# pyranha-labs/hypergrep

Hardware: NVIDIA B200
Metric: scanned GB/s (higher is better)
Workload: dtype u8

## Files before the change

### hypergrep_b200/csrc/capi.cpp

```cpp
#include <cuda_runtime.h>
#include <sys/stat.h>

#include <algorithm>
#include <atomic>
#include <chrono>
#include <cstdio>
#include <cstdlib>
#include <cstring>
#include <condition_variable>
#include <functional>
#include <list>
#include <mutex>
#include <thread>
#include <utility>
#include <string>
#include <vector>

#include "../../include/gpugrep.h"
#include "database.hpp"
#include "engine.hpp"
#include "ingest.hpp"

namespace gpugrep {
void set_last_error(const std::string& e);
// ... 240 lines not shown
    std::vector<uint32_t> report_end_flat;

    bool limit_reached() const { return max_match > 0 && out->count() >= max_match; }

    int deliver(const SegmentResult& r, const uint8_t* host, ScanSlot* slot) {
        stats.lines += r.num_lines;
        stats.gpu_ms += r.stats.gpu_ms;
        stats.stream_kernel_ms += r.stats.stream_ms;
        stats.launches += r.stats.launches;
        stats.stream_launches += r.stats.stream_launches;
        stats.candidates += r.stats.candidates;
        stats.h2d_bytes += r.stats.h2d_bytes;
        stats.d2h_bytes += r.stats.d2h_bytes;
        stats.path |= r.stats.path;
        stats.segments++;
        if (stop) return 0;
        int rc = db->simple ? deliver_simple(r, host, slot) : deliver_events(r, host, slot);
        line_base += r.num_lines;
        return rc;
    }

    int deliver_simple(const SegmentResult& r, const uint8_t* host, ScanSlot* slot) {
        const LineRec* recs = r.lines;
        size_t count = r.num_line_recs;
        const bool fast_rec = (r.stats.path & 1) != 0;
        if (fast_rec) {
            if (!out->wants_lines() && max_match == 0) { out->emit_count_only(r.num_valid_recs); return 0; }
            if (r.num_valid_recs != count) {
                unique_.clear();
                unique_.reserve(r.num_valid_recs);
// ... 578 lines not shown
            spec.count_only = count_only;
            std::memset(&stats[g], 0, sizeof(gpugrep_stats));
            rcs[g] = spec.end > spec.begin ? run(g, spec, &stats[g]) : 0;
            if (rcs[g]) errors[g] = gpugrep_last_error();
        });
    }
    for (auto& w : workers) w.join();
    gpugrep_stats total;
    std::memset(&total, 0, sizeof(total));
    for (size_t g = 0; g < G; g++) {
        if (rcs[g]) { set_last_error(errors[g]); return rcs[g]; }
        total.bytes_scanned += stats[g].bytes_scanned; total.lines += stats[g].lines; total.candidates += stats[g].candidates;
        total.h2d_bytes += stats[g].h2d_bytes; total.d2h_bytes += stats[g].d2h_bytes; total.gpu_ms += stats[g].gpu_ms;
        total.stream_kernel_ms += stats[g].stream_kernel_ms; total.launches += stats[g].launches;
        total.stream_launches += stats[g].stream_launches; total.segments += stats[g].segments; total.path |= stats[g].path;
    }
    Deliverer out(pr.cb, effective_batch(pr));
    unsigned long long line_base = 0;
    bool stop = false;
    for (size_t g = 0; g < G && !stop; g++) {
        if (count_only) {
            out.emit_count_only(stats[g].matches);
        } else {
            const auto& recs = results[g].records;
            for (size_t i = 0; i < recs.size() && !stop;) {
                size_t j = i;
                for (; j < recs.size() && recs[j].line == recs[i].line; j++) {
                    if (pr.cb) out.emit_text(recs[j].id, line_base + recs[j].line, results[g].text.data() + recs[j].offset);
                    else out.emit_count_only(1);
                }
// ... 169 lines not shown
```

### hypergrep_b200/csrc/device_types.cuh

```cuda
#pragma once

namespace gpugrep {

struct GroupDev {
    const uint16_t* trans;
    const uint8_t* cls;
    const uint32_t* accept_of;
    const uint16_t* flat;
    const uint16_t* eod_next;
    const uint16_t* ctab;
    const uint8_t* cmap;
    uint32_t crow, cstates;
    const uint8_t* depth;
    uint32_t cdepth_off;
    uint32_t stride, eod, first_accept, dead, accept_base, idle_end, mid_other, mid_word;
};

struct DbView {
    const GroupDev* groups;
    int ngroups;
    const NfaView* nfas;
    int nnfa;
};

constexpr uint32_t kInvalidLen = 0xffffffffu;
constexpr uint32_t kHasNulBit = 0x80000000u;

struct Totals {
    unsigned long long meta_total;
    unsigned long long rec_total;
    unsigned long long aux_total;
    unsigned int flags;
    unsigned int last_byte;
    unsigned int max_line;
    unsigned int survivors;
};

#define CUDA_TRY(expr)                                                                      \
    do {                                                                                    \
        cudaError_t e_ = (expr);                                                            \
        if (e_ != cudaSuccess) {                                                            \
// ... 7 lines not shown
```

### hypergrep_b200/csrc/engine.cu

```cuda
#include <cuda_runtime.h>

#include <algorithm>
#include <cstdio>
#include <cstdlib>
#include <cstring>
#include <mutex>
#include <unordered_map>
#include <vector>

#include "engine.hpp"
#include "nfa_sim.hpp"

#include "device_types.cuh"
#include "swar.cuh"
#include "confirm.cuh"
#include "k_stream.cuh"
#include "scan.cuh"
#include "dfa_walk.cuh"
#include "k_fast.cuh"
#include "k_general.cuh"
#include "k_invert.cuh"

namespace gpugrep {

// ... 399 lines not shown
}

template <class Load>
static void launch_scan(cudaStream_t st, Load load, size_t n, unsigned long long* out, unsigned long long* sums, unsigned long long* total,
                        SegmentStats& stats, const unsigned long long* limit = nullptr, int limit_shift = 32) {
    size_t nb = (n + kScanTile - 1) / kScanTile;
    if (nb == 0) nb = 1;
    static const unsigned per_sm = blocks_per_sm(k_scan_sums<Load>, kScanThreads);
    unsigned grid = (unsigned)std::min<size_t>(nb, (size_t)per_sm * device_sms());
    k_scan_sums<Load><<<grid, kScanThreads, 0, st>>>(load, n, sums, nb, limit, limit_shift);
    k_scan_top<<<1, 1024, 0, st>>>(sums, nb, total);
    k_scan_write<Load><<<grid, kScanThreads, 0, st>>>(load, n, sums, out, nb, limit, limit_shift);
    stats.launches += 3;
}

template <int STRIDE, bool FOLD, int MODE, int NODD = 0>
static cudaError_t launch_stream_t(cudaStream_t st, int grid, int block, size_t smem, const uint8_t* data, size_t n, unsigned long long* meta,
                                   uint32_t* nlmask, unsigned long long* gsum, const DevicePrefilter* pf) {
    if (smem > 48 * 1024) {
        cudaError_t e = cudaFuncSetAttribute(k_stream<STRIDE, FOLD, MODE, NODD>, cudaFuncAttributeMaxDynamicSharedMemorySize, (int)smem);
        if (e != cudaSuccess) return e;
    }
    k_stream<STRIDE, FOLD, MODE, NODD><<<grid, block, smem, st>>>(data, n, meta, nlmask, gsum, pf ? pf->d_table : nullptr, pf ? pf->table_words : 0,
                                                            pf ? pf->pp : ProbeParams{});
    return cudaGetLastError();
}

template <int MODE>
static cudaError_t launch_stream_m(cudaStream_t st, int grid, int block, size_t smem, const uint8_t* data, size_t n, unsigned long long* meta,
                                   uint32_t* nlmask, unsigned long long* gsum, const DevicePrefilter* pf) {
    int key = pf->stride * 2 + (pf->fold ? 1 : 0);
    if (MODE == 2 && pf->stride == 4 && pf->nodd > 0)
        return pf->fold ? launch_stream_t<4, true, MODE, 2>(st, grid, block, smem, data, n, meta, nlmask, gsum, pf)
                        : launch_stream_t<4, false, MODE, 2>(st, grid, block, smem, data, n, meta, nlmask, gsum, pf);
    switch (key) {
        case 8: return launch_stream_t<4, false, MODE>(st, grid, block, smem, data, n, meta, nlmask, gsum, pf);
        case 9: return launch_stream_t<4, true, MODE>(st, grid, block, smem, data, n, meta, nlmask, gsum, pf);
        case 4: return launch_stream_t<2, false, MODE>(st, grid, block, smem, data, n, meta, nlmask, gsum, pf);
        case 5: return launch_stream_t<2, true, MODE>(st, grid, block, smem, data, n, meta, nlmask, gsum, pf);
        case 2: return launch_stream_t<1, false, MODE>(st, grid, block, smem, data, n, meta, nlmask, gsum, pf);
        default: return launch_stream_t<1, true, MODE>(st, grid, block, smem, data, n, meta, nlmask, gsum, pf);
    }
}

int slot_submit(ScanSlot* s, const DeviceDb& ddb, const DevicePrefilter* pf, const uint8_t* host_data, const uint8_t* dev_data, size_t n,
                int buffer_size, void* user_stream, std::string& error) {
    if (n >= ((size_t)1 << 32) - 1024) { error = "segment too large"; return 7; }
    s->stream = user_stream ? (cudaStream_t)user_stream : s->own_stream;
    cudaStream_t st = s->stream;
    s->ddb = &ddb;
    s->n = n;
    s->buffer_size = buffer_size;
    s->stats = SegmentStats();
    s->nblk = (n + 511) / 512;
    size_t super_bytes = 0;
    if (buffer_size >= 4096) {
// ... 64 lines not shown
    size_t smem = 0;
    if (s->fast) smem = (size_t)pf->table_words * 4 + (pf->mode == 1 ? pf->pp.half_bytes : 0);
    int block = smem > 32 * 1024 ? 1024 : 256;
    int ctas_per_sm = smem > 100 * 1024 ? 1 : (smem > 32 * 1024 ? 2 : 6);
    int grid = device_sms() * ctas_per_sm;
    size_t groups = (s->nblk + kStreamU - 1) / kStreamU;
    size_t max_grid = (groups + (block / 32) - 1) / (block / 32);
    if ((size_t)grid > max_grid) grid = (int)std::max<size_t>(1, max_grid);
    unsigned long long* meta = s->d_meta.as<unsigned long long>();
    uint32_t* nlmask = s->d_nlmask.as<uint32_t>();
    unsigned long long* gsum = s->d_gsum.as<unsigned long long>();
    const size_t ngroups = (s->nblk + kGroupBlocks - 1) / kGroupBlocks;
    CUDA_TRY(cudaMemsetAsync(gsum + (ngroups ? ngroups - 1 : 0), 0, 16, st));
    CUDA_TRY(cudaEventRecord(s->ev[2], st));
    cudaError_t le;
    if (!s->fast) le = launch_stream_t<4, false, 0>(st, grid, block, 0, s->data, n, meta, nlmask, gsum, nullptr);
    else if (pf->mode == 1) le = launch_stream_m<1>(st, grid, block, smem, s->data, n, meta, nlmask, gsum, pf);
    else le = launch_stream_m<2>(st, grid, block, smem, s->data, n, meta, nlmask, gsum, pf);
    if (le != cudaSuccess) { error = std::string("k_stream launch: ") + cudaGetErrorString(le); return 7; }
    CUDA_TRY(cudaEventRecord(s->ev[3], st));
    s->stats.launches++;
    s->stats.stream_launches++;
    unsigned long long* prefix = s->d_prefix.as<unsigned long long>();
    launch_scan(st, LoadU64{gsum}, ngroups, prefix, s->d_sums.as<unsigned long long>(), &dT->meta_total, s->stats);
    if (s->fast) {
        const unsigned sms = (unsigned)device_sms();
        const size_t bps = super_bytes / 512;
        static const unsigned list_per_sm = blocks_per_sm(k_list_candidates, 256);
        k_list_candidates<<<(unsigned)std::min<size_t>((s->nblk + 255) / 256, (size_t)list_per_sm * sms), 256, 0, st>>>(meta, prefix, s->nblk, bps, &dT->meta_total,
                                                                                                                    s->d_cand.as<uint32_t>(), s->cand_cap, dT);
        DbView view{ddb.d_groups, ddb.ngroups, ddb.d_nfas, ddb.nnfa};
        uint32_t* tile_records = s->d_recoff.as<uint32_t>();
        CUDA_TRY(cudaMemsetAsync(tile_records, 0, (s->cand_cap / kEmitTile + 2) * sizeof(uint32_t), st));
// ... 19 lines not shown
        if (!v1 && ddb.smem_table_bytes && hitinfo == nullptr && pf->lookback <= 64u) {
            const size_t vsmem = 256 + ddb.smem_table_bytes;
            CUDA_TRY(cudaFuncSetAttribute(k_verify_smem, cudaFuncAttributeMaxDynamicSharedMemorySize, (int)vsmem));
            const unsigned per_sm = blocks_per_sm(k_verify_smem, kVerifySmemThreads, vsmem);
            unsigned vgrid = (unsigned)std::min<size_t>((s->cand_cap + kVerifySmemThreads - 1) / kVerifySmemThreads, (size_t)per_sm * sms);
            k_verify_smem<<<vgrid, kVerifySmemThreads, vsmem, st>>>(view, s->data, n, s->d_cand.as<uint32_t>(), &dT->meta_total, s->cand_cap, pf->lookback,
                                                                    idle_span, s->d_res.as<uint32_t>(), tile_records);
        } else {
            auto kernel = ddb.nnfa > 0 ? k_verify_local<true> : k_verify_local<false>;
            const unsigned verify_per_sm = blocks_per_sm(kernel, 128);
            unsigned vgrid = (unsigned)std::min<size_t>((s->cand_cap + 127) / 128, (size_t)verify_per_sm * sms);
            kernel<<<vgrid, 128, 0, st>>>(view, s->data, n, s->d_cand.as<uint32_t>(), &dT->meta_total, s->cand_cap, pf->lookback, idle_span, hitinfo,
                                          survivors, dT, s->d_res.as<uint32_t>(), tile_records);
        }
        k_tile_offsets<<<1, 1024, 0, st>>>(tile_records, &dT->meta_total, s->cand_cap, &dT->rec_total);
        auto emit_kernel = ddb.nnfa > 0 ? k_emit_nlm<true> : k_emit_nlm<false>;
        const unsigned emit_per_sm = blocks_per_sm(emit_kernel, kEmitThreads);
        emit_kernel<<<(unsigned)std::min<size_t>((s->cand_cap + kEmitTile - 1) / kEmitTile, (size_t)emit_per_sm * sms), kEmitThreads, 0, st>>>(
            view, s->data, n, s->d_cand.as<uint32_t>(), s->d_res.as<uint32_t>(), tile_records, meta, prefix, nlmask, &dT->meta_total,
            s->cand_cap, s->d_recs.as<LineRec>(), s->rec_cap, dT);
        k_dedupe_records<<<(unsigned)std::min<size_t>((s->rec_cap + 255) / 256, (size_t)sms * 4), 256, 0, st>>>(s->d_recs.as<LineRec>(), s->rec_cap, dT);
        s->stats.launches += 5;
        CUDA_TRY(cudaEventRecord(s->ev[1], st));
    }
    CUDA_TRY(cudaMemcpyAsync(&dT->last_byte, s->data + n - 1, 1, cudaMemcpyDeviceToDevice, st));
    CUDA_TRY(cudaMemcpyAsync(s->h_totals.p, dT, sizeof(Totals), cudaMemcpyDeviceToHost, st));
    CUDA_TRY(cudaEventRecord(s->done, st));
    CUDA_TRY(cudaGetLastError());
    return 0;
}

int ScanSlot::run_general(SegmentResult& out, std::string& error) {
    cudaStream_t st = stream;
    Totals* dT = d_totals.as<Totals>();
    Totals* hT = h_totals.as<Totals>();
    stats.path |= 2;
// ... 120 lines not shown
    CUDA_TRY(cudaEventRecord(ev[1], st));
    CUDA_TRY(cudaMemcpyAsync(h_recs.p, d_invrecs.p, selected * sizeof(LineRec), cudaMemcpyDeviceToHost, st));
    CUDA_TRY(cudaStreamSynchronize(st));
    CUDA_TRY(cudaGetLastError());
    stats.d2h_bytes += selected * sizeof(LineRec);
    return 0;
}

int slot_collect(ScanSlot* s, SegmentResult& out, std::string& error, size_t split_above) {
    cudaStream_t st = s->stream;
    out = SegmentResult();
    CUDA_TRY(cudaEventSynchronize(s->done));
    s->stats.d2h_bytes += sizeof(Totals);
    if (s->n == 0) { out.stats = s->stats; return 0; }
    Totals* hT = s->h_totals.as<Totals>();
    bool done = false;
    if (s->fast) {
        s->stats.candidates = hT->meta_total >> 32;
        if (hT->flags == 0) {
            s->stats.path |= 1;
            size_t nrec = (size_t)hT->rec_total;
            out.num_valid_recs = (size_t)hT->aux_total;
            const size_t nl_total = (size_t)(uint32_t)hT->meta_total;
            out.num_lines = nl_total + ((hT->last_byte & 0xff) != '\n' ? 1 : 0);
            if (s->invert) {
                const size_t selected = (size_t)out.num_lines - out.num_valid_recs;
                if (selected && s->want_records) {
                    int rc = s->run_complement(nrec, (size_t)out.num_lines, selected, error);
                    if (rc) return rc;
                }
                nrec = selected;
                out.num_valid_recs = selected;
            } else if (nrec && s->want_records) {
                if (s->h_recs.reserve(nrec * sizeof(LineRec)) != cudaSuccess) { error = "cudaHostAlloc failed"; return 3; }
// ... 76 lines not shown
```

### hypergrep_b200/csrc/engine.hpp

```cpp
#pragma once
#include <cstddef>
#include <cstdint>
#include <memory>
#include <string>
#include <vector>

#include "database.hpp"

namespace gpugrep {

struct LineRec {
    uint32_t line;
    uint32_t start;
    uint32_t len;
};
constexpr uint32_t kLineLenMask = 0x7fffffffu;
constexpr uint32_t kLineHasNul = 0x80000000u;
constexpr uint32_t kLineInvalid = 0xffffffffu;

struct EventRec {
    uint32_t line, start, len;
    uint32_t end;
    uint32_t report;
};

struct SegmentStats {
    double gpu_ms = 0, stream_ms = 0;
    unsigned launches = 0, stream_launches = 0;
    unsigned long long candidates = 0;
    unsigned long long h2d_bytes = 0, d2h_bytes = 0;
    unsigned path = 0;
};

struct SegmentResult {
    uint64_t num_lines = 0;
    const LineRec* lines = nullptr;
    size_t num_line_recs = 0;
    size_t num_valid_recs = 0;
    const EventRec* events = nullptr;
    size_t num_events = 0;
    SegmentStats stats;
};

struct DeviceDb;
struct DevicePrefilter;
class ScanSlot;
// ... 31 lines not shown
```

### hypergrep_b200/csrc/k_fast.cuh

```cuda
#pragma once

namespace gpugrep {

__global__ void k_list_candidates(const unsigned long long* __restrict__ meta, const unsigned long long* __restrict__ prefix, size_t nblk,
                                  size_t blocks_per_super, const unsigned long long* meta_total, uint32_t* __restrict__ cand, size_t cap,
                                  Totals* totals) {
    const size_t ngroups = (nblk + kGroupBlocks - 1) / kGroupBlocks;
    for (size_t grp = (size_t)blockIdx.x * blockDim.x + threadIdx.x; grp < ngroups; grp += (size_t)gridDim.x * blockDim.x) {
        const unsigned long long before = prefix[grp];
        const size_t first = grp * kGroupBlocks;
        if (blocks_per_super && first % blocks_per_super == 0 && first + blocks_per_super <= nblk) {
            const size_t hi = first + blocks_per_super;
            const uint32_t b = hi < nblk ? (uint32_t)prefix[hi / kGroupBlocks] : (uint32_t)*meta_total;
            if ((uint32_t)before == b) atomicOr(&totals->flags, 1u);
        }
        size_t at = (size_t)(before >> 32);
        for (size_t g = first; g < nblk && g < first + kGroupBlocks; g++) {
            uint32_t mask = (uint32_t)meta[g];
            while (mask) {
                int b = __ffs(mask) - 1;
                mask &= mask - 1;
                if (at < cap) cand[at] = (uint32_t)(g * 32 + b);
                else atomicOr(&totals->flags, 2u);
                at++;
// ... 435 lines not shown
        bool nul = false;
#pragma unroll
        for (int j = 0; j < 4; j++) {
            const uint32_t cb = pos + 512u * j + 16u * lane;
            if (cb < to) {
                uint32_t zm = byte_mask16(v[j], 0u);
                if (cb + 16u > to) zm &= (1u << (to - cb)) - 1u;
                nul |= zm != 0u;
            }
        }
        if (__any_sync(0xffffffffu, nul)) return true;
    }
    return false;
}

constexpr uint32_t kNulBound = 512;
template <bool WITH_NFA>
__device__ uint32_t emit_lane_nlm(const DbView& db, const uint8_t* __restrict__ data, size_t n, const uint32_t* __restrict__ cand,
                                  const uint32_t* __restrict__ marks, const unsigned long long* __restrict__ meta,
                                  const unsigned long long* __restrict__ prefix, const uint32_t* __restrict__ nlmask, uint32_t nblk, bool live, size_t i,
                                  size_t at, LineRec* __restrict__ recs, size_t rec_cap, Totals* totals) {
    const uint32_t lane = threadIdx.x & 31;
    uint32_t valid = 0;
    uint32_t mask = live ? marks[i] : 0u;
    const uint32_t o = live ? cand[i] * 16u : 0u;
    uint32_t nlm = 0;
    if (live && ((nlmask[o >> 9] >> ((o >> 4) & 31u)) & 1u)) nlm = newline_mask16(ld_chunk(data, o, n));
    uint32_t st = 0;
    bool first = true;
    while (__any_sync(0xffffffffu, mask != 0)) {
        while (mask != 0 && !(mask & 1u)) {
            if (!nlm) { mask = 0; break; }
            st = o + __ffs(nlm);
            nlm &= nlm - 1;
            first = false;
            mask >>= 1;
        }
        const bool work = mask != 0;
        uint32_t en = 0, resume = 0;
        bool has_nul = false, settled = true, ok = true;
        if (work) {
            if (first) st = nlm_line_start(data, n, nlmask, o);
            en = nlm ? o + __ffs(nlm) : nlm_line_end(data, n, nlmask, nblk, o + 16u < (uint32_t)n ? o + 16u : (uint32_t)n - 1u);
            settled = nul_scan_bounded(data, n, st, en, kNulBound, &has_nul, &resume);
        }
        for (uint32_t pend = __ballot_sync(0xffffffffu, work && !settled); pend; pend &= pend - 1) {
            const int src = __ffs(pend) - 1;
            const bool more = warp_nul_scan(data, n, __shfl_sync(0xffffffffu, resume, src), __shfl_sync(0xffffffffu, en, src));
            if ((int)lane == src) has_nul = more;
        }
        if (work) {
            if (ok && has_nul) ok = block_matches<false>(db, data, st, en) || (WITH_NFA && block_matches_nfa(db, data, st, en));
            valid += ok ? 1u : 0u;
            const uint32_t line_no = nlm_line_number(data, meta, prefix, nlmask, st);
            if (at < rec_cap) recs[at] = LineRec{line_no, st, ok ? ((en - st) | (has_nul ? kHasNulBit : 0u)) : kInvalidLen};
            else atomicOr(&totals->flags, 4u);
            at++;
            if (!nlm) mask = 0;
            else {
                st = o + __ffs(nlm);
                nlm &= nlm - 1;
                first = false;
                mask >>= 1;
            }
        }
    }
    return valid;
}

template <bool WITH_NFA>
__global__ void __launch_bounds__(kEmitThreads, 6) k_emit_nlm(DbView db, const uint8_t* __restrict__ data, size_t n, const uint32_t* __restrict__ cand,
                                                           const uint32_t* __restrict__ marks, const uint32_t* __restrict__ tile_offsets,
                                                           const unsigned long long* __restrict__ meta, const unsigned long long* __restrict__ prefix,
                                                           const uint32_t* __restrict__ nlmask, const unsigned long long* meta_total, size_t cap,
                                                           LineRec* __restrict__ recs, size_t rec_cap, Totals* totals) {
    __shared__ uint32_t q_cand[kEmitQueue], q_at[kEmitQueue];
    __shared__ unsigned long long s_warp[kEmitThreads / 32], s_total;
    const uint32_t nblk = (uint32_t)((n + 511) >> 9);
    uint32_t valid = 0;
    uint32_t head = 0, queued = 0;
    size_t ncand = (size_t)(*meta_total >> 32);
    if (ncand > cap) ncand = cap;
    constexpr int kPer = kEmitTile / kEmitThreads;
    const size_t ntiles = (ncand + kEmitTile - 1) / kEmitTile;
    for (size_t block_base = (size_t)blockIdx.x * kEmitTile; block_base < ncand; block_base += (size_t)gridDim.x * kEmitTile) {
        {
            const size_t tile = block_base / kEmitTile;
            const uint32_t next = tile + 1 < ntiles ? tile_offsets[tile + 1] : (uint32_t)totals->rec_total;
            if (next == tile_offsets[tile]) continue;
        }
        uint32_t mk[kPer];
        uint32_t records = 0, marked = 0;
#pragma unroll
// ... 7 lines not shown
        uint32_t slot = head + queued + (uint32_t)(before >> 32);
        uint32_t at = tile_offsets[block_base / kEmitTile] + (uint32_t)before;
#pragma unroll
        for (int j = 0; j < kPer; j++) {
            if (mk[j]) {
                q_cand[slot & (kEmitQueue - 1)] = (uint32_t)(block_base + (size_t)threadIdx.x * kPer + j);
                q_at[slot & (kEmitQueue - 1)] = at;
                slot++;
                at += __popc(mk[j]);
            }
        }
        queued += (uint32_t)(s_total >> 32);
        __syncthreads();
        while (queued >= (uint32_t)kEmitThreads) {
            const uint32_t k = (head + threadIdx.x) & (kEmitQueue - 1);
            valid += emit_lane_nlm<WITH_NFA>(db, data, n, cand, marks, meta, prefix, nlmask, nblk, true, q_cand[k], q_at[k], recs, rec_cap, totals);
            head += kEmitThreads;
            queued -= kEmitThreads;
        }
        __syncthreads();
    }
    if (queued) {
        constexpr uint32_t kWarps = kEmitThreads / 32;
        const uint32_t j = (threadIdx.x >> 5) + kWarps * (threadIdx.x & 31);
        const uint32_t k = (head + j) & (kEmitQueue - 1);
        const bool live = j < queued;
        valid += emit_lane_nlm<WITH_NFA>(db, data, n, cand, marks, meta, prefix, nlmask, nblk, live, live ? q_cand[k] : 0, live ? q_at[k] : 0, recs, rec_cap, totals);
    }
    (void)valid;
}

__global__ void __launch_bounds__(256) k_dedupe_records(LineRec* __restrict__ recs, size_t rec_cap, Totals* totals) {
    size_t nrec = (size_t)totals->rec_total;
    if (nrec > rec_cap) nrec = rec_cap;
    uint32_t valid = 0;
    for (size_t i = (size_t)blockIdx.x * blockDim.x + threadIdx.x; i < nrec; i += (size_t)gridDim.x * blockDim.x) {
        if (i > 0 && recs[i].start == recs[i - 1].start) recs[i].len = kInvalidLen;
        else if (recs[i].len != kInvalidLen) valid++;
    }
    valid = __reduce_add_sync(0xffffffffu, valid);
    if ((threadIdx.x & 31) == 0 && valid) atomicAdd(&totals->aux_total, (unsigned long long)valid);
}

__global__ void k_find_cuts(const uint8_t* __restrict__ data, size_t size, size_t chunk, size_t window, size_t ncuts, unsigned long long* __restrict__ cuts) {
    size_t j = (size_t)blockIdx.x * blockDim.x + threadIdx.x;
    if (j >= ncuts) return;
    size_t b = (j + 1) * chunk;
    if (b >= size) { cuts[j] = size; return; }
    size_t lo = b > window ? b - window : 0;
    unsigned long long found = 0;
    for (size_t p = b; p > lo; p--) {
        if ((p & 15) == 0 && data[p - 1] == '\n') { found = p; break; }
    }
// ... 5 lines not shown
```

### hypergrep_b200/csrc/k_stream.cuh

```cuda
#pragma once

namespace gpugrep {

__device__ __forceinline__ uint32_t lds32(uint32_t shared_addr) {
    uint32_t v;
    asm("ld.shared.u32 %0, [%1];" : "=r"(v) : "r"(shared_addr));
    return v;
}

__device__ __forceinline__ uint32_t lds8(uint32_t shared_addr) {
    uint32_t v;
    asm("ld.shared.u8 %0, [%1];" : "=r"(v) : "r"(shared_addr));
    return v;
}

template <int STRIDE, bool FOLD, int MODE, int NODD>
__device__ __forceinline__ bool probe_chunk(const uint4& v, uint32_t next, const uint32_t* __restrict__ tab, const ProbeParams& pp, uint32_t c1,
                                            uint32_t c2) {
    if (MODE == 0) return false;
    uint32_t w[5] = {v.x, v.y, v.z, v.w, next};
    if (FOLD) {
#pragma unroll
        for (int i = 0; i < 5; i++) w[i] |= 0x20202020u;
    }
// ... 26 lines not shown
        }
        return (MODE == 1 ? false : (bits & 1u) != 0u) || miss == 0u;
    }
    return MODE == 1 ? miss == 0u : (bits & 1u) != 0u;
}

__device__ __forceinline__ uint32_t newline_count16_fma(const uint4& v, uint32_t cnl, uint32_t c80) {
    uint32_t a = eq_mask4_r(v.x, cnl, c80), b = eq_mask4_r(v.y, cnl, c80), c = eq_mask4_r(v.z, cnl, c80), d = eq_mask4_r(v.w, cnl, c80);
    unsigned long long acc = a;
    asm("mad.wide.u32 %0, %1, 2, %0;" : "+l"(acc) : "r"(b));
    asm("mad.wide.u32 %0, %1, 4, %0;" : "+l"(acc) : "r"(c));
    asm("mad.wide.u32 %0, %1, 8, %0;" : "+l"(acc) : "r"(d));
    return __popcll(acc);
}

constexpr int kStreamU = 4;

struct StreamRegs {
    uint32_t c1, c2, cnl, c80, lane;
};

template <int STRIDE, bool FOLD, int MODE, int NODD>
__device__ __forceinline__ void stream_group(const uint4 (&v)[kStreamU], uint32_t g0, const uint8_t* __restrict__ data, size_t n,
                                             unsigned long long* __restrict__ meta, uint32_t* __restrict__ nlmask, unsigned long long* __restrict__ gsum,
                                             const uint32_t* __restrict__ s_tab, const ProbeParams& pp, const StreamRegs& r) {
    constexpr int U = kStreamU;
    const uint32_t lane = r.lane;
    uint32_t after = 0;
    if (MODE != 0 && (STRIDE < 4 || NODD > 0) && lane == 31) {
        size_t off = (size_t)(g0 + U) << 9;
        if (off + 4 <= n) after = *reinterpret_cast<const uint32_t*>(data + off);
        else if (off < n) after = ld_chunk(data, off, n).x;
    }
    uint32_t cnt01, cnt23, masks[U], nlm[U];
    {
        uint32_t c[U];
#pragma unroll
        for (int u = 0; u < U; u++) {
            c[u] = newline_count16_fma(v[u], r.cnl, r.c80);
            nlm[u] = __ballot_sync(0xffffffffu, c[u] != 0u);
            uint32_t nx = 0;
            if (MODE != 0 && (STRIDE < 4 || NODD > 0)) {
                uint32_t give = (u + 1 < U && lane == 0) ? v[u + 1 < U ? u + 1 : u].x : v[u].x;
                nx = __shfl_sync(0xffffffffu, give, (lane + 1) & 31);
                if (u + 1 == U && lane == 31) nx = after;
            }
            bool hit = probe_chunk<STRIDE, FOLD, MODE, NODD>(v[u], nx, s_tab, pp, r.c1, r.c2);
            masks[u] = __ballot_sync(0xffffffffu, hit);
        }
        cnt01 = __reduce_add_sync(0xffffffffu, c[0] | (c[1] << 16));
        cnt23 = __reduce_add_sync(0xffffffffu, c[2] | (c[3] << 16));
    }
    if (lane == 0) {
        uint4* out = reinterpret_cast<uint4*>(meta + g0);
        out[0] = make_uint4(masks[0], cnt01 & 0xffffu, masks[1], cnt01 >> 16);
        out[1] = make_uint4(masks[2], cnt23 & 0xffffu, masks[3], cnt23 >> 16);
        *reinterpret_cast<uint4*>(nlmask + g0) = make_uint4(nlm[0], nlm[1], nlm[2], nlm[3]);
        const uint32_t cands = __popc(masks[0]) + __popc(masks[1]) + __popc(masks[2]) + __popc(masks[3]);
        const uint32_t sum = cnt01 + cnt23;
        gsum[g0 / U] = ((unsigned long long)cands << 32) | ((sum & 0xffffu) + (sum >> 16));
    }
}

template <int STRIDE, bool FOLD, int MODE, int NODD>
__global__ void __launch_bounds__(1024) k_stream(const uint8_t* __restrict__ data, size_t n, unsigned long long* __restrict__ meta,
                                                 uint32_t* __restrict__ nlmask, unsigned long long* __restrict__ gsum,
                                                 const uint32_t* __restrict__ table, int table_words, ProbeParams pp) {
    extern __shared__ __align__(16) uint32_t s_raw[];
    uint32_t* s_tab = s_raw;
    uint32_t saddr = (uint32_t)__cvta_generic_to_shared(s_raw);
    if (MODE == 1) {
        uint32_t aligned = (saddr + pp.half_bytes - 1u) & ~(pp.half_bytes - 1u);
        s_tab = s_raw + ((aligned - saddr) >> 2);
        saddr = aligned;
    }
    if (MODE != 0) {
        for (int i = threadIdx.x; i < table_words; i += blockDim.x) s_tab[i] = table[i];
        __syncthreads();
    }
    constexpr int U = kStreamU;
    StreamRegs r;
    r.lane = threadIdx.x & 31;
    const uint32_t lane = r.lane;
    const uint32_t replica4 = (lane & ((1u << pp.rshift) - 1u)) << 2;
    r.c1 = MODE == 1 ? (saddr | replica4) : saddr;
    r.c2 = (saddr + pp.half_bytes) | replica4;
    asm volatile("mov.u32 %0, %0;" : "+r"(r.c1));
    asm volatile("mov.u32 %0, %0;" : "+r"(r.c2));
    asm volatile("mov.u32 %0, 0x0a0a0a0a;" : "=r"(r.cnl));
    asm volatile("mov.u32 %0, 0x80808080;" : "=r"(r.c80));
    const uint32_t warp = (blockIdx.x * blockDim.x + threadIdx.x) >> 5;
    const uint32_t nwarps = (gridDim.x * blockDim.x) >> 5;
    const uint32_t nblk = (uint32_t)((n + 511) >> 9);
    const uint32_t nfull = (uint32_t)(n >> 9);
    const uint32_t step = nwarps * U;

    uint4 ahead[U];
    const uint8_t* lane_data = data + lane * 16;
    if (warp * U + U <= nfull) {
#pragma unroll
        for (int u = 0; u < U; u++) ahead[u] = ld_stream16(lane_data + ((size_t)(warp * U) << 9) + u * 512);
    }
    for (uint32_t g0 = warp * U; g0 + U <= nfull; g0 += step) {
        uint4 v[U];
#pragma unroll
        for (int u = 0; u < U; u++) v[u] = ahead[u];
        const uint32_t g1 = g0 + step;
        if (g1 + U <= nfull) {
#pragma unroll
            for (int u = 0; u < U; u++) ahead[u] = ld_stream16(lane_data + ((size_t)g1 << 9) + u * 512);
        }
        stream_group<STRIDE, FOLD, MODE, NODD>(v, g0, data, n, meta, nlmask, gsum, s_tab, pp, r);
    }

    const uint32_t tail0 = (nfull / U) * U;
    for (uint32_t g = tail0 + warp; g < nblk; g += nwarps) {
        size_t off = ((size_t)g << 9) + (size_t)lane * 16;
        uint4 v = off < n ? ld_chunk(data, off, n) : make_uint4(0, 0, 0, 0);
        uint32_t nx = 0;
        if (MODE != 0 && (STRIDE < 4 || NODD > 0)) {
            nx = __shfl_down_sync(0xffffffffu, v.x, 1);
            if (lane == 31) {
                size_t o2 = (size_t)(g + 1) << 9;
                nx = o2 < n ? ld_chunk(data, o2, n).x : 0u;
            }
        }
        uint32_t cnt = newline_count16_fma(v, r.cnl, r.c80);
        bool hit = probe_chunk<STRIDE, FOLD, MODE, NODD>(v, nx, s_tab, pp, r.c1, r.c2);
        if (off >= n) hit = false;
        uint32_t mask = __ballot_sync(0xffffffffu, hit);
        uint32_t nl = __ballot_sync(0xffffffffu, cnt != 0u);
        uint32_t total = __reduce_add_sync(0xffffffffu, cnt);
        if (lane == 0) {
            meta[g] = ((unsigned long long)total << 32) | mask;
            nlmask[g] = nl;
            atomicAdd(&gsum[tail0 / U], ((unsigned long long)__popc(mask) << 32) | total);
        }
    }
}

}
```

### hypergrep_b200/utils.py

```python

from __future__ import annotations

import ctypes
import os
import re
import threading
from typing import Callable, Sequence

HS_FLAG_CASELESS = 1
HS_FLAG_DOTALL = 2
HS_FLAG_MULTILINE = 4
HS_FLAG_SINGLEMATCH = 8
_DEFAULT_FLAGS = HS_FLAG_DOTALL | HS_FLAG_MULTILINE | HS_FLAG_SINGLEMATCH

RC_INVALID_FILE = 101
_RC_INTERRUPTED = 130

_LIB_NAME = "libgpugrep.so"
_lock = threading.Lock()
_state: dict = {"lib": None, "libzstd": None, "libhs": None}


class Result(ctypes.Structure):

# ... 118 lines not shown
    worker.start()
    try:
        worker.join(timeout=3600)
    except KeyboardInterrupt:
        outcome["rc"] = _RC_INTERRUPTED
    return outcome["rc"]


class _Stats(ctypes.Structure):

    _fields_ = [
        ("bytes_scanned", ctypes.c_ulonglong), ("lines", ctypes.c_ulonglong), ("matches", ctypes.c_ulonglong),
        ("candidates", ctypes.c_ulonglong), ("h2d_bytes", ctypes.c_ulonglong), ("d2h_bytes", ctypes.c_ulonglong),
        ("gpu_ms", ctypes.c_double), ("stream_kernel_ms", ctypes.c_double), ("wall_ms", ctypes.c_double),
        ("launches", ctypes.c_uint), ("stream_launches", ctypes.c_uint), ("segments", ctypes.c_uint), ("path", ctypes.c_uint),
        ("split_segments", ctypes.c_uint), ("reserved", ctypes.c_uint),
    ]


_FILE_ENTRY_ARGTYPES = [ctypes.c_char_p, ctypes.c_void_p, ctypes.c_void_p, ctypes.c_void_p, ctypes.c_uint, ctypes.c_void_p,
                        ctypes.c_int, ctypes.c_int, ctypes.c_ulonglong, ctypes.c_void_p]


def _invert_entry(lib: ctypes.CDLL):
    try:
        entry = lib.gpugrep_invert_scan_file
    except AttributeError as error:
        raise NotImplementedError(
            "invert_match needs gpugrep_invert_scan_file, which the loaded native library does not export "
            f"({_library_path()}); there is no CPU fallback"
        ) from error
# ... 164 lines not shown
```

### include/gpugrep.h

```cpp
#ifndef GPUGREP_H
#define GPUGREP_H

#include <stddef.h>
#include <stdint.h>

#if defined(__GNUC__)
#define GPUGREP_API __attribute__((visibility("default")))
#else
#define GPUGREP_API
#endif

#ifdef __cplusplus
extern "C" {
#endif


enum gpugrep_ret {
    GPUGREP_OK = 0,
    GPUGREP_COMPILE_MEM = 1,
    GPUGREP_COMPILE = 2,
    GPUGREP_SCRATCH = 3,
    GPUGREP_DB = 4,
    GPUGREP_STATE_MEM = 5,
    GPUGREP_GZ_OPEN = 6,
// ... 19 lines not shown
typedef struct gpugrep_stats {
    unsigned long long bytes_scanned;
    unsigned long long lines;
    unsigned long long matches;
    unsigned long long candidates;
    unsigned long long h2d_bytes;
    unsigned long long d2h_bytes;
    double gpu_ms;
    double stream_kernel_ms;
    double wall_ms;
    unsigned int launches;
    unsigned int stream_launches;
    unsigned int segments;
    unsigned int path;
    unsigned int split_segments;
    unsigned int reserved;
} gpugrep_stats;

#define GPUGREP_LOC_HOST 0
#define GPUGREP_LOC_DEVICE 1

GPUGREP_API int gpugrep_scan_buffer(const void* data, size_t size, int location, const char* const* patterns,
                        const unsigned int* pattern_flags, const unsigned int* pattern_ids, unsigned int elements,
                        hs_event on_event, int buffer_size, int buffer_count, unsigned long long max_match_count,
                        void* stream, gpugrep_stats* stats);

GPUGREP_API int gpugrep_scan_file(const char* file_name, const char* const* patterns, const unsigned int* pattern_flags,
                      const unsigned int* pattern_ids, unsigned int elements, hs_event on_event, int buffer_size,
                      int buffer_count, unsigned long long max_match_count, gpugrep_stats* stats);

GPUGREP_API int gpugrep_invert_scan_file(const char* file_name, const char* const* patterns, const unsigned int* pattern_flags,
// ... 86 lines not shown
```

Before: 2205.

## Detect NUL-free segments in stream kernel and add count-only emit path

When records are not wanted, the stream kernel now accumulates a per-segment NUL-byte flag with SWAR arithmetic. The emit kernel uses it to skip per-line NUL scanning and line-number computation, writing only a 32-bit line key per match. A new key-counting kernel replaces record dedupe in count-only mode, which shrinks output traffic and avoids the line-start/line-end walks. The cost is extra ALU work in the streaming hot loop, more template instantiations, and a new flag bit that has to be masked out of the fallback check.

```diff
diff --git a/hypergrep_b200/csrc/capi.cpp b/hypergrep_b200/csrc/capi.cpp
--- a/hypergrep_b200/csrc/capi.cpp
+++ b/hypergrep_b200/csrc/capi.cpp
@@ -278,6 +278,7 @@
         stats.d2h_bytes += r.stats.d2h_bytes;
         stats.path |= r.stats.path;
         stats.segments++;
+        stats.nul_segments += r.stats.nul ? 1u : 0u;
         if (stop) return 0;
         int rc = db->simple ? deliver_simple(r, host, slot) : deliver_events(r, host, slot);
         line_base += r.num_lines;
@@ -886,6 +887,7 @@
         total.h2d_bytes += stats[g].h2d_bytes; total.d2h_bytes += stats[g].d2h_bytes; total.gpu_ms += stats[g].gpu_ms;
         total.stream_kernel_ms += stats[g].stream_kernel_ms; total.launches += stats[g].launches;
         total.stream_launches += stats[g].stream_launches; total.segments += stats[g].segments; total.path |= stats[g].path;
+        total.nul_segments += stats[g].nul_segments;
     }
     Deliverer out(pr.cb, effective_batch(pr));
     unsigned long long line_base = 0;
diff --git a/hypergrep_b200/csrc/device_types.cuh b/hypergrep_b200/csrc/device_types.cuh
--- a/hypergrep_b200/csrc/device_types.cuh
+++ b/hypergrep_b200/csrc/device_types.cuh
@@ -25,6 +25,8 @@
 
 constexpr uint32_t kInvalidLen = 0xffffffffu;
 constexpr uint32_t kHasNulBit = 0x80000000u;
+constexpr unsigned int kFallbackFlags = 7u;
+constexpr unsigned int kSegmentNulFlag = 8u;
 
 struct Totals {
     unsigned long long meta_total;
diff --git a/hypergrep_b200/csrc/engine.cu b/hypergrep_b200/csrc/engine.cu
--- a/hypergrep_b200/csrc/engine.cu
+++ b/hypergrep_b200/csrc/engine.cu
@@ -437,32 +437,34 @@
     stats.launches += 3;
 }
 
-template <int STRIDE, bool FOLD, int MODE, int NODD = 0>
+template <int STRIDE, bool FOLD, int MODE, int NODD, bool NUL>
 static cudaError_t launch_stream_t(cudaStream_t st, int grid, int block, size_t smem, const uint8_t* data, size_t n, unsigned long long* meta,
-                                   uint32_t* nlmask, unsigned long long* gsum, const DevicePrefilter* pf) {
+                                   uint32_t* nlmask, unsigned long long* gsum, const DevicePrefilter* pf,
+                                   unsigned int* flags) {
     if (smem > 48 * 1024) {
-        cudaError_t e = cudaFuncSetAttribute(k_stream<STRIDE, FOLD, MODE, NODD>, cudaFuncAttributeMaxDynamicSharedMemorySize, (int)smem);
+        cudaError_t e = cudaFuncSetAttribute(k_stream<STRIDE, FOLD, MODE, NODD, NUL>, cudaFuncAttributeMaxDynamicSharedMemorySize, (int)smem);
         if (e != cudaSuccess) return e;
     }
-    k_stream<STRIDE, FOLD, MODE, NODD><<<grid, block, smem, st>>>(data, n, meta, nlmask, gsum, pf ? pf->d_table : nullptr, pf ? pf->table_words : 0,
-                                                            pf ? pf->pp : ProbeParams{});
+    k_stream<STRIDE, FOLD, MODE, NODD, NUL><<<grid, block, smem, st>>>(data, n, meta, nlmask, gsum, pf ? pf->d_table : nullptr, pf ? pf->table_words : 0,
+                                                            pf ? pf->pp : ProbeParams{}, flags);
     return cudaGetLastError();
 }
 
-template <int MODE>
+template <int MODE, bool NUL>
 static cudaError_t launch_stream_m(cudaStream_t st, int grid, int block, size_t smem, const uint8_t* data, size_t n, unsigned long long* meta,
-                                   uint32_t* nlmask, unsigned long long* gsum, const DevicePrefilter* pf) {
+                                   uint32_t* nlmask, unsigned long long* gsum, const DevicePrefilter* pf,
+                                   unsigned int* flags) {
     int key = pf->stride * 2 + (pf->fold ? 1 : 0);
     if (MODE == 2 && pf->stride == 4 && pf->nodd > 0)
-        return pf->fold ? launch_stream_t<4, true, MODE, 2>(st, grid, block, smem, data, n, meta, nlmask, gsum, pf)
-                        : launch_stream_t<4, false, MODE, 2>(st, grid, block, smem, data, n, meta, nlmask, gsum, pf);
+        return pf->fold ? launch_stream_t<4, true, MODE, 2, NUL>(st, grid, block, smem, data, n, meta, nlmask, gsum, pf, flags)
+                        : launch_stream_t<4, false, MODE, 2, NUL>(st, grid, block, smem, data, n, meta, nlmask, gsum, pf, flags);
     switch (key) {
-        case 8: return launch_stream_t<4, false, MODE>(st, grid, block, smem, data, n, meta, nlmask, gsum, pf);
-        case 9: return launch_stream_t<4, true, MODE>(st, grid, block, smem, data, n, meta, nlmask, gsum, pf);
-        case 4: return launch_stream_t<2, false, MODE>(st, grid, block, smem, data, n, meta, nlmask, gsum, pf);
-        case 5: return launch_stream_t<2, true, MODE>(st, grid, block, smem, data, n, meta, nlmask, gsum, pf);
-        case 2: return launch_stream_t<1, false, MODE>(st, grid, block, smem, data, n, meta, nlmask, gsum, pf);
-        default: return launch_stream_t<1, true, MODE>(st, grid, block, smem, data, n, meta, nlmask, gsum, pf);
+        case 8: return launch_stream_t<4, false, MODE, 0, NUL>(st, grid, block, smem, data, n, meta, nlmask, gsum, pf, flags);
+        case 9: return launch_stream_t<4, true, MODE, 0, NUL>(st, grid, block, smem, data, n, meta, nlmask, gsum, pf, flags);
+        case 4: return launch_stream_t<2, false, MODE, 0, NUL>(st, grid, block, smem, data, n, meta, nlmask, gsum, pf, flags);
+        case 5: return launch_stream_t<2, true, MODE, 0, NUL>(st, grid, block, smem, data, n, meta, nlmask, gsum, pf, flags);
+        case 2: return launch_stream_t<1, false, MODE, 0, NUL>(st, grid, block, smem, data, n, meta, nlmask, gsum, pf, flags);
+        default: return launch_stream_t<1, true, MODE, 0, NUL>(st, grid, block, smem, data, n, meta, nlmask, gsum, pf, flags);
     }
 }
 
@@ -557,9 +559,13 @@
     CUDA_TRY(cudaMemsetAsync(gsum + (ngroups ? ngroups - 1 : 0), 0, 16, st));
     CUDA_TRY(cudaEventRecord(s->ev[2], st));
     cudaError_t le;
-    if (!s->fast) le = launch_stream_t<4, false, 0>(st, grid, block, 0, s->data, n, meta, nlmask, gsum, nullptr);
-    else if (pf->mode == 1) le = launch_stream_m<1>(st, grid, block, smem, s->data, n, meta, nlmask, gsum, pf);
-    else le = launch_stream_m<2>(st, grid, block, smem, s->data, n, meta, nlmask, gsum, pf);
+    const bool nul_test = !s->want_records;
+    if (!s->fast) le = nul_test ? launch_stream_t<4, false, 0, 0, true>(st, grid, block, 0, s->data, n, meta, nlmask, gsum, nullptr, &dT->flags)
+                                : launch_stream_t<4, false, 0, 0, false>(st, grid, block, 0, s->data, n, meta, nlmask, gsum, nullptr, &dT->flags);
+    else if (pf->mode == 1) le = nul_test ? launch_stream_m<1, true>(st, grid, block, smem, s->data, n, meta, nlmask, gsum, pf, &dT->flags)
+                                          : launch_stream_m<1, false>(st, grid, block, smem, s->data, n, meta, nlmask, gsum, pf, &dT->flags);
+    else le = nul_test ? launch_stream_m<2, true>(st, grid, block, smem, s->data, n, meta, nlmask, gsum, pf, &dT->flags)
+                       : launch_stream_m<2, false>(st, grid, block, smem, s->data, n, meta, nlmask, gsum, pf, &dT->flags);
     if (le != cudaSuccess) { error = std::string("k_stream launch: ") + cudaGetErrorString(le); return 7; }
     CUDA_TRY(cudaEventRecord(s->ev[3], st));
     s->stats.launches++;
@@ -609,12 +615,18 @@
                                           survivors, dT, s->d_res.as<uint32_t>(), tile_records);
         }
         k_tile_offsets<<<1, 1024, 0, st>>>(tile_records, &dT->meta_total, s->cand_cap, &dT->rec_total);
-        auto emit_kernel = ddb.nnfa > 0 ? k_emit_nlm<true> : k_emit_nlm<false>;
+        const bool count_only = !s->want_records;
+        auto emit_kernel = ddb.nnfa > 0 ? (count_only ? k_emit_nlm<true, true> : k_emit_nlm<true, false>)
+                                        : (count_only ? k_emit_nlm<false, true> : k_emit_nlm<false, false>);
+        const size_t out_cap = count_only ? s->rec_cap * sizeof(LineRec) / sizeof(uint32_t) : s->rec_cap;
         const unsigned emit_per_sm = blocks_per_sm(emit_kernel, kEmitThreads);
         emit_kernel<<<(unsigned)std::min<size_t>((s->cand_cap + kEmitTile - 1) / kEmitTile, (size_t)emit_per_sm * sms), kEmitThreads, 0, st>>>(
             view, s->data, n, s->d_cand.as<uint32_t>(), s->d_res.as<uint32_t>(), tile_records, meta, prefix, nlmask, &dT->meta_total,
-            s->cand_cap, s->d_recs.as<LineRec>(), s->rec_cap, dT);
-        k_dedupe_records<<<(unsigned)std::min<size_t>((s->rec_cap + 255) / 256, (size_t)sms * 4), 256, 0, st>>>(s->d_recs.as<LineRec>(), s->rec_cap, dT);
+            s->cand_cap, s->d_recs.as<LineRec>(), s->d_recs.as<uint32_t>(), out_cap, dT);
+        if (count_only)
+            k_count_keys<<<(unsigned)std::min<size_t>((out_cap + 255) / 256, (size_t)sms * 4), 256, 0, st>>>(s->d_recs.as<uint32_t>(), out_cap, dT);
+        else
+            k_dedupe_records<<<(unsigned)std::min<size_t>((s->rec_cap + 255) / 256, (size_t)sms * 4), 256, 0, st>>>(s->d_recs.as<LineRec>(), s->rec_cap, dT);
         s->stats.launches += 5;
         CUDA_TRY(cudaEventRecord(s->ev[1], st));
     }
@@ -765,10 +777,11 @@
     s->stats.d2h_bytes += sizeof(Totals);
     if (s->n == 0) { out.stats = s->stats; return 0; }
     Totals* hT = s->h_totals.as<Totals>();
+    s->stats.nul = (hT->flags & kSegmentNulFlag) != 0;
     bool done = false;
     if (s->fast) {
         s->stats.candidates = hT->meta_total >> 32;
-        if (hT->flags == 0) {
+        if ((hT->flags & kFallbackFlags) == 0) {
             s->stats.path |= 1;
             size_t nrec = (size_t)hT->rec_total;
             out.num_valid_recs = (size_t)hT->aux_total;
diff --git a/hypergrep_b200/csrc/engine.hpp b/hypergrep_b200/csrc/engine.hpp
--- a/hypergrep_b200/csrc/engine.hpp
+++ b/hypergrep_b200/csrc/engine.hpp
@@ -30,6 +30,7 @@
     unsigned long long candidates = 0;
     unsigned long long h2d_bytes = 0, d2h_bytes = 0;
     unsigned path = 0;
+    bool nul = false;
 };
 
 struct SegmentResult {
diff --git a/hypergrep_b200/csrc/k_fast.cuh b/hypergrep_b200/csrc/k_fast.cuh
--- a/hypergrep_b200/csrc/k_fast.cuh
+++ b/hypergrep_b200/csrc/k_fast.cuh
@@ -473,12 +473,30 @@
     return false;
 }
 
+constexpr uint32_t kNoNewlineKey = 0xfffffffeu;
+__device__ uint32_t nlm_line_key(const uint32_t* __restrict__ nlmask, uint32_t o) {
+    const uint32_t c = o >> 4;
+    uint32_t b = c >> 5;
+    uint32_t w = nlmask[b] & ((1u << (c & 31u)) - 1u);
+    while (true) {
+        if (w) return (b * 32u + (31u - __clz(w))) * 16u + 15u;
+        if (b == 0) return kNoNewlineKey;
+        if (b >= 4) {
+            const uint32_t w3 = nlmask[b - 1], w2 = nlmask[b - 2], w1 = nlmask[b - 3], w0 = nlmask[b - 4];
+            if (w3) { b -= 1; w = w3; } else if (w2) { b -= 2; w = w2; } else if (w1) { b -= 3; w = w1; } else { b -= 4; w = w0; }
+        } else {
+            b--;
+            w = nlmask[b];
+        }
+    }
+}
+
 constexpr uint32_t kNulBound = 512;
-template <bool WITH_NFA>
+template <bool WITH_NFA, bool COUNT_ONLY>
 __device__ uint32_t emit_lane_nlm(const DbView& db, const uint8_t* __restrict__ data, size_t n, const uint32_t* __restrict__ cand,
                                   const uint32_t* __restrict__ marks, const unsigned long long* __restrict__ meta,
                                   const unsigned long long* __restrict__ prefix, const uint32_t* __restrict__ nlmask, uint32_t nblk, bool live, size_t i,
-                                  size_t at, LineRec* __restrict__ recs, size_t rec_cap, Totals* totals) {
+                                  size_t at, LineRec* __restrict__ recs, uint32_t* __restrict__ keys, size_t rec_cap, bool nul_free, Totals* totals) {
     const uint32_t lane = threadIdx.x & 31;
     uint32_t valid = 0;
     uint32_t mask = live ? marks[i] : 0u;
@@ -487,6 +505,30 @@
     if (live && ((nlmask[o >> 9] >> ((o >> 4) & 31u)) & 1u)) nlm = newline_mask16(ld_chunk(data, o, n));
     uint32_t st = 0;
     bool first = true;
+    if (COUNT_ONLY && nul_free) {
+        const uint32_t key_base = (o >> 4) * 16u + 15u;
+        while (mask != 0) {
+            while (!(mask & 1u)) {
+                if (!nlm) { mask = 0; break; }
+                nlm &= nlm - 1;
+                first = false;
+                mask >>= 1;
+            }
+            if (mask == 0) break;
+            const uint32_t key = first ? nlm_line_key(nlmask, o) : key_base - __popc(nlm);
+            valid++;
+            if (at < rec_cap) keys[at] = key;
+            else atomicOr(&totals->flags, 4u);
+            at++;
+            if (!nlm) mask = 0;
+            else {
+                nlm &= nlm - 1;
+                first = false;
+                mask >>= 1;
+            }
+        }
+        return valid;
+    }
     while (__any_sync(0xffffffffu, mask != 0)) {
         while (mask != 0 && !(mask & 1u)) {
             if (!nlm) { mask = 0; break; }
@@ -501,7 +543,7 @@
         if (work) {
             if (first) st = nlm_line_start(data, n, nlmask, o);
             en = nlm ? o + __ffs(nlm) : nlm_line_end(data, n, nlmask, nblk, o + 16u < (uint32_t)n ? o + 16u : (uint32_t)n - 1u);
-            settled = nul_scan_bounded(data, n, st, en, kNulBound, &has_nul, &resume);
+            if (!nul_free) settled = nul_scan_bounded(data, n, st, en, kNulBound, &has_nul, &resume);
         }
         for (uint32_t pend = __ballot_sync(0xffffffffu, work && !settled); pend; pend &= pend - 1) {
             const int src = __ffs(pend) - 1;
@@ -511,9 +553,14 @@
         if (work) {
             if (ok && has_nul) ok = block_matches<false>(db, data, st, en) || (WITH_NFA && block_matches_nfa(db, data, st, en));
             valid += ok ? 1u : 0u;
-            const uint32_t line_no = nlm_line_number(data, meta, prefix, nlmask, st);
-            if (at < rec_cap) recs[at] = LineRec{line_no, st, ok ? ((en - st) | (has_nul ? kHasNulBit : 0u)) : kInvalidLen};
-            else atomicOr(&totals->flags, 4u);
+            if (COUNT_ONLY) {
+                if (at < rec_cap) keys[at] = ok ? st : kInvalidLen;
+                else atomicOr(&totals->flags, 4u);
+            } else {
+                const uint32_t line_no = nlm_line_number(data, meta, prefix, nlmask, st);
+                if (at < rec_cap) recs[at] = LineRec{line_no, st, ok ? ((en - st) | (has_nul ? kHasNulBit : 0u)) : kInvalidLen};
+                else atomicOr(&totals->flags, 4u);
+            }
             at++;
             if (!nlm) mask = 0;
             else {
@@ -527,15 +574,16 @@
     return valid;
 }
 
-template <bool WITH_NFA>
+template <bool WITH_NFA, bool COUNT_ONLY>
 __global__ void __launch_bounds__(kEmitThreads, 6) k_emit_nlm(DbView db, const uint8_t* __restrict__ data, size_t n, const uint32_t* __restrict__ cand,
                                                            const uint32_t* __restrict__ marks, const uint32_t* __restrict__ tile_offsets,
                                                            const unsigned long long* __restrict__ meta, const unsigned long long* __restrict__ prefix,
                                                            const uint32_t* __restrict__ nlmask, const unsigned long long* meta_total, size_t cap,
-                                                           LineRec* __restrict__ recs, size_t rec_cap, Totals* totals) {
+                                                           LineRec* __restrict__ recs, uint32_t* __restrict__ keys, size_t rec_cap, Totals* totals) {
     __shared__ uint32_t q_cand[kEmitQueue], q_at[kEmitQueue];
     __shared__ unsigned long long s_warp[kEmitThreads / 32], s_total;
     const uint32_t nblk = (uint32_t)((n + 511) >> 9);
+    const bool nul_free = COUNT_ONLY && !(totals->flags & kSegmentNulFlag);
     uint32_t valid = 0;
     uint32_t head = 0, queued = 0;
     size_t ncand = (size_t)(*meta_total >> 32);
@@ -573,7 +621,8 @@
         __syncthreads();
         while (queued >= (uint32_t)kEmitThreads) {
             const uint32_t k = (head + threadIdx.x) & (kEmitQueue - 1);
-            valid += emit_lane_nlm<WITH_NFA>(db, data, n, cand, marks, meta, prefix, nlmask, nblk, true, q_cand[k], q_at[k], recs, rec_cap, totals);
+            valid += emit_lane_nlm<WITH_NFA, COUNT_ONLY>(db, data, n, cand, marks, meta, prefix, nlmask, nblk, true, q_cand[k], q_at[k], recs, keys, rec_cap,
+                                                                 nul_free, totals);
             head += kEmitThreads;
             queued -= kEmitThreads;
         }
@@ -584,7 +633,8 @@
         const uint32_t j = (threadIdx.x >> 5) + kWarps * (threadIdx.x & 31);
         const uint32_t k = (head + j) & (kEmitQueue - 1);
         const bool live = j < queued;
-        valid += emit_lane_nlm<WITH_NFA>(db, data, n, cand, marks, meta, prefix, nlmask, nblk, live, live ? q_cand[k] : 0, live ? q_at[k] : 0, recs, rec_cap, totals);
+        valid += emit_lane_nlm<WITH_NFA, COUNT_ONLY>(db, data, n, cand, marks, meta, prefix, nlmask, nblk, live, live ? q_cand[k] : 0, live ? q_at[k] : 0,
+                                                             recs, keys, rec_cap, nul_free, totals);
     }
     (void)valid;
 }
@@ -596,6 +646,18 @@
     for (size_t i = (size_t)blockIdx.x * blockDim.x + threadIdx.x; i < nrec; i += (size_t)gridDim.x * blockDim.x) {
         if (i > 0 && recs[i].start == recs[i - 1].start) recs[i].len = kInvalidLen;
         else if (recs[i].len != kInvalidLen) valid++;
+    }
+    valid = __reduce_add_sync(0xffffffffu, valid);
+    if ((threadIdx.x & 31) == 0 && valid) atomicAdd(&totals->aux_total, (unsigned long long)valid);
+}
+
+__global__ void __launch_bounds__(256) k_count_keys(const uint32_t* __restrict__ keys, size_t cap, Totals* totals) {
+    size_t nkeys = (size_t)totals->rec_total;
+    if (nkeys > cap) nkeys = cap;
+    uint32_t valid = 0;
+    for (size_t i = (size_t)blockIdx.x * blockDim.x + threadIdx.x; i < nkeys; i += (size_t)gridDim.x * blockDim.x) {
+        const uint32_t key = keys[i];
+        if (key != kInvalidLen && (i == 0 || key != keys[i - 1])) valid++;
     }
     valid = __reduce_add_sync(0xffffffffu, valid);
     if ((threadIdx.x & 31) == 0 && valid) atomicAdd(&totals->aux_total, (unsigned long long)valid);
diff --git a/hypergrep_b200/csrc/k_stream.cuh b/hypergrep_b200/csrc/k_stream.cuh
--- a/hypergrep_b200/csrc/k_stream.cuh
+++ b/hypergrep_b200/csrc/k_stream.cuh
@@ -64,16 +64,26 @@
     return __popcll(acc);
 }
 
+__device__ __forceinline__ void nul_accumulate(const uint4& v, uint32_t& acc) {
+    const uint32_t w[4] = {v.x, v.y, v.z, v.w};
+#pragma unroll
+    for (int i = 0; i < 4; i++) {
+        uint32_t t;
+        asm("mad.lo.u32 %0, %1, 1, 0xfefefeff;" : "=r"(t) : "r"(w[i]));
+        asm("lop3.b32 %0, %1, %2, %0, 0xBA;" : "+r"(acc) : "r"(t), "r"(w[i]));
+    }
+}
+
 constexpr int kStreamU = 4;
 
 struct StreamRegs {
     uint32_t c1, c2, cnl, c80, lane;
 };
 
-template <int STRIDE, bool FOLD, int MODE, int NODD>
+template <int STRIDE, bool FOLD, int MODE, int NODD, bool NUL>
 __device__ __forceinline__ void stream_group(const uint4 (&v)[kStreamU], uint32_t g0, const uint8_t* __restrict__ data, size_t n,
                                              unsigned long long* __restrict__ meta, uint32_t* __restrict__ nlmask, unsigned long long* __restrict__ gsum,
-                                             const uint32_t* __restrict__ s_tab, const ProbeParams& pp, const StreamRegs& r) {
+                                             const uint32_t* __restrict__ s_tab, const ProbeParams& pp, const StreamRegs& r, uint32_t& nul) {
     constexpr int U = kStreamU;
     const uint32_t lane = r.lane;
     uint32_t after = 0;
@@ -88,6 +98,7 @@
 #pragma unroll
         for (int u = 0; u < U; u++) {
             c[u] = newline_count16_fma(v[u], r.cnl, r.c80);
+            if (NUL) nul_accumulate(v[u], nul);
             nlm[u] = __ballot_sync(0xffffffffu, c[u] != 0u);
             uint32_t nx = 0;
             if (MODE != 0 && (STRIDE < 4 || NODD > 0)) {
@@ -112,10 +123,11 @@
     }
 }
 
-template <int STRIDE, bool FOLD, int MODE, int NODD>
+template <int STRIDE, bool FOLD, int MODE, int NODD, bool NUL>
 __global__ void __launch_bounds__(1024) k_stream(const uint8_t* __restrict__ data, size_t n, unsigned long long* __restrict__ meta,
                                                  uint32_t* __restrict__ nlmask, unsigned long long* __restrict__ gsum,
-                                                 const uint32_t* __restrict__ table, int table_words, ProbeParams pp) {
+                                                 const uint32_t* __restrict__ table, int table_words, ProbeParams pp,
+                                                 unsigned int* __restrict__ flags) {
     extern __shared__ __align__(16) uint32_t s_raw[];
     uint32_t* s_tab = s_raw;
     uint32_t saddr = (uint32_t)__cvta_generic_to_shared(s_raw);
@@ -144,6 +156,7 @@
     const uint32_t nblk = (uint32_t)((n + 511) >> 9);
     const uint32_t nfull = (uint32_t)(n >> 9);
     const uint32_t step = nwarps * U;
+    uint32_t nul = 0;
 
     uint4 ahead[U];
     const uint8_t* lane_data = data + lane * 16;
@@ -160,10 +173,11 @@
 #pragma unroll
             for (int u = 0; u < U; u++) ahead[u] = ld_stream16(lane_data + ((size_t)g1 << 9) + u * 512);
         }
-        stream_group<STRIDE, FOLD, MODE, NODD>(v, g0, data, n, meta, nlmask, gsum, s_tab, pp, r);
+        stream_group<STRIDE, FOLD, MODE, NODD, NUL>(v, g0, data, n, meta, nlmask, gsum, s_tab, pp, r, nul);
     }
 
     const uint32_t tail0 = (nfull / U) * U;
+    bool tail_nul = false;
     for (uint32_t g = tail0 + warp; g < nblk; g += nwarps) {
         size_t off = ((size_t)g << 9) + (size_t)lane * 16;
         uint4 v = off < n ? ld_chunk(data, off, n) : make_uint4(0, 0, 0, 0);
@@ -178,6 +192,10 @@
         uint32_t cnt = newline_count16_fma(v, r.cnl, r.c80);
         bool hit = probe_chunk<STRIDE, FOLD, MODE, NODD>(v, nx, s_tab, pp, r.c1, r.c2);
         if (off >= n) hit = false;
+        if (NUL) {
+            const uint32_t inside = off >= n ? 0u : (off + 16 > n ? (1u << (uint32_t)(n - off)) - 1u : 0xffffu);
+            tail_nul |= (byte_mask16(v, 0u) & inside) != 0u;
+        }
         uint32_t mask = __ballot_sync(0xffffffffu, hit);
         uint32_t nl = __ballot_sync(0xffffffffu, cnt != 0u);
         uint32_t total = __reduce_add_sync(0xffffffffu, cnt);
@@ -187,6 +205,7 @@
             atomicAdd(&gsum[tail0 / U], ((unsigned long long)__popc(mask) << 32) | total);
         }
     }
-}
-
-}
+    if (NUL && __any_sync(0xffffffffu, (nul & 0x80808080u) != 0u || tail_nul) && lane == 0) atomicOr(flags, kSegmentNulFlag);
+}
+
+}
diff --git a/hypergrep_b200/utils.py b/hypergrep_b200/utils.py
--- a/hypergrep_b200/utils.py
+++ b/hypergrep_b200/utils.py
@@ -156,7 +156,7 @@
         ("candidates", ctypes.c_ulonglong), ("h2d_bytes", ctypes.c_ulonglong), ("d2h_bytes", ctypes.c_ulonglong),
         ("gpu_ms", ctypes.c_double), ("stream_kernel_ms", ctypes.c_double), ("wall_ms", ctypes.c_double),
         ("launches", ctypes.c_uint), ("stream_launches", ctypes.c_uint), ("segments", ctypes.c_uint), ("path", ctypes.c_uint),
-        ("split_segments", ctypes.c_uint), ("reserved", ctypes.c_uint),
+        ("split_segments", ctypes.c_uint), ("nul_segments", ctypes.c_uint),
     ]
 
 
diff --git a/include/gpugrep.h b/include/gpugrep.h
--- a/include/gpugrep.h
+++ b/include/gpugrep.h
@@ -57,7 +57,7 @@
     unsigned int segments;
     unsigned int path;
     unsigned int split_segments;
-    unsigned int reserved;
+    unsigned int nul_segments;
 } gpugrep_stats;
 
 #define GPUGREP_LOC_HOST 0
```

Result: faster. 2398, median of 6 (+8.8%).
